# Pearbiossom-M/FlashAttention-from-Scratch-with-Triton

Measured on AMD Instinct MI355X. Metric: achieved TFLOPS fwd and fwd+bwd (B=4,H=32,N=4096,D=64 causal); %MFMA peak, higher is better.
Workload: dtype bf16

## Files before the change

### flashattention-from-scratch-with-triton_amd/csrc/fa_fwd_v4.hip

```cpp
#include <stdlib.h>

#include <type_traits>

#include "fa_common.h"
#include "fa_kernels.h"

namespace fa {

template <int D_>
struct Fwd4Cfg {
  static constexpr int D = D_;
  static constexpr int BM = 256, NT = 256, NW = 4;
  static constexpr int BN = D == 64 ? 128 : 64;
  static constexpr int NBUF = D == 64 ? 3 : 4;
  static constexpr int NKB = BN / 32;
  static constexpr int ROWB = D * 2, CPR = D / 8, KS = D / 16, DB = D / 32;
  static constexpr int TILE_BYTES = BN * ROWB;
  static constexpr int V_BASE = NBUF * TILE_BYTES;
  static constexpr int FLAG_OFF = 2 * NBUF * TILE_BYTES;
  static constexpr int RB_BYTES = 32 * ROWB;
  static constexpr int QS_OFF = FLAG_OFF + 16;
  static constexpr int QS_BYTES = D == 64 ? 8 * RB_BYTES : 0;
  static constexpr int LDS_BYTES = QS_OFF + QS_BYTES;
  static constexpr int PIECES = TILE_BYTES / (NW * 1024);
  static constexpr int RPI = 1024 / ROWB;
  static constexpr int PVG = 2 * DB;
  static constexpr int NSS = 2 * KS, NPV = 2 * PVG, NSLOT = NSS + NPV;
  static constexpr int INFLIGHT = (NBUF - 3) * 2 * PIECES;
};

template <typename T> struct Fwd4Limit;
template <> struct Fwd4Limit<BF16> { static constexpr float value = 1.2676506e30f; };
template <> struct Fwd4Limit<FP16> { static constexpr float value = 32768.0f; };

#ifdef FA_STAMPS
#define FA4_STAMP(slot)                                                           \
  do {                                                                            \
    __builtin_amdgcn_sched_barrier(0);                                            \
    unsigned long long now_;                                                      \
    asm volatile("s_memtime %0\n\ts_waitcnt lgkmcnt(0)" : "=s"(now_)::"memory"); \
    __builtin_amdgcn_sched_barrier(0);                                            \
    seg[slot] += now_ - last_;                                                    \
    last_ = now_;                                                                 \
  } while (0)
#else
#define FA4_STAMP(slot) do {} while (0)
#endif

template <int D, typename T, bool CAUSAL>
__global__ __launch_bounds__(256, 1) void fa_fwd4_kernel(FwdParams p) {
#ifdef FA_STAMPS
  unsigned long long clk0_, rt0_;
  asm volatile("s_memtime %0\n\ts_memrealtime %1\n\ts_waitcnt lgkmcnt(0)" : "=s"(clk0_), "=s"(rt0_)::"memory");
  unsigned long long seg[12] = {0, 0, 0, 0, 0, 0, 0, 0, 0, 0, 0, 0};
  unsigned long long last_ = clk0_, ntile_ = 0, npass_ = 0;
#endif
  using C = Fwd4Cfg<D>;
  using vec8 = typename T::vec8;
  constexpr bool FOLD = T::kFoldScale;
  constexpr bool CHAIN_M = FOLD;
  extern __shared__ __attribute__((aligned(16))) char smem_raw[];
  FA_LDS char* smem = (FA_LDS char*)smem_raw;

  const int tid = threadIdx.x;
  const int lane = tid & 63;
  const int wave = __builtin_amdgcn_readfirstlane(tid >> 6);
  const int r = lane & 31, h = lane >> 5;

  const bool CONT = CAUSAL || (p.Sk % C::BN == 0 && p.Sk / C::BN >= C::NBUF - 1);
  constexpr bool STAGEQ = D == 64;
  const bool paired = CAUSAL && p.pair;
  const int nq = p.nq_tiles;
  const int per_bh = paired ? (nq + 1) / 2 : nq;
  const int n_items = per_bh * p.B * p.H;
  const int Sq = p.Sq, Sk = p.Sk;
  struct Work {
    int b, h, idx, npass;
  };
  auto decode = [&](int item) __attribute__((always_inline)) -> Work {
    const int w = xcd_remap(item, n_items);
    const int bh = p.div_per_bh.div(w), idx = w - bh * per_bh, b = p.div_h.div(bh);
    return Work{b, bh - b * p.H, idx, (paired && idx != nq - 1 - idx) ? 2 : 1};
  };
  auto tile_of = [&](const Work& wk, int pass) __attribute__((always_inline)) -> int {
    return paired ? (pass == 0 ? nq - 1 - wk.idx : wk.idx) : (CAUSAL ? nq - 1 - wk.idx : wk.idx);
  };

  const int q_rs = p.lq.rs, kv_rs = p.lk.rs, o_rs = p.lo.rs;
  auto rsrc_q = [&](const Work& wk, bool valid) __attribute__((always_inline)) {
    return make_rsrc((const char*)p.q + wk.b * p.lq.sb + wk.h * p.lq.sh, valid ? view_bytes(Sq, q_rs, C::ROWB) : 0u);
  };
  auto rsrc_k = [&](const Work& wk, bool valid) __attribute__((always_inline)) {
    return make_rsrc((const char*)p.k + wk.b * p.lk.sb + wk.h * p.lk.sh, valid ? view_bytes(Sk, kv_rs, C::ROWB) : 0u);
  };
  auto rsrc_v = [&](const Work& wk, bool valid) __attribute__((always_inline)) {
    return make_rsrc((const char*)p.v + wk.b * p.lv.sb + wk.h * p.lv.sh, valid ? view_bytes(Sk, kv_rs, C::ROWB) : 0u);
  };

  int dma_src[C::PIECES];
#pragma unroll
  for (int i = 0; i < C::PIECES; ++i) {
    const int row = (C::BN / C::NW) * wave + C::RPI * i + lane / C::CPR;
    dma_src[i] = row * kv_rs + swz_chunk<D>(row, lane % C::CPR) * 16 - 1024 * (i & 1);
  }
  int k_off[C::KS];
#pragma unroll
  for (int ks = 0; ks < C::KS; ++ks) k_off[ks] = lds_off<D>(r, 2 * ks + h);
  int v_off[2][C::DB];
#pragma unroll
  for (int e = 0; e < 2; ++e)
#pragma unroll
    for (int db = 0; db < C::DB; ++db) v_off[e][db] = tr_lane_off<D>(lane, 8 * e, db);
  const float c2 = p.scale * kLog2e;

  if (Sk % C::BN != 0) {
    lds_zero_fill(smem, C::FLAG_OFF, C::NT, tid);
    __syncthreads();
  }

  if (tid == 0) *(FA_LDS int*)(smem + C::FLAG_OFF) = 0;
  bool primed = false;
  int r0 = 0;

  int item = blockIdx.x, pass = 0;
  Work wk = decode(item);
  Work nwk_item = decode(min(item + (int)gridDim.x, n_items - 1));
  for (;;) {
    const int b_ = wk.b, h_ = wk.h;
    const __amdgpu_buffer_rsrc_t rk = rsrc_k(wk, true), rv = rsrc_v(wk, true);
    const __amdgpu_buffer_rsrc_t ro = make_rsrc((char*)p.o + b_ * p.lo.sb + h_ * p.lo.sh, view_bytes(Sq, o_rs, C::ROWB));
    const __amdgpu_buffer_rsrc_t rl = make_rsrc(p.lse + b_ * p.lse_sb + h_ * p.lse_sh, (unsigned)Sq * 4);
    const bool more_pass = pass + 1 < wk.npass, more_item = item + (int)gridDim.x < n_items;
    const bool has_next = CONT && (more_pass || more_item);
    const Work nwk = more_pass ? wk : nwk_item;
    const int nq0_wg = tile_of(nwk, more_pass ? pass + 1 : 0) * C::BM;

    FA4_STAMP(8);
    const int q0_wg = tile_of(wk, pass) * C::BM;
    const int qw = q0_wg + 32 * wave;
    auto qrow = [&](int rb) __attribute__((always_inline)) { return qw + 128 * rb; };

    const int kv_end = CAUSAL ? min(Sk, q0_wg + C::BM) : Sk;
    const int ntiles = (kv_end + C::BN - 1) / C::BN;
    const int nplain = CAUSAL ? min(Sk / C::BN, q0_wg / C::BN) : Sk / C::BN;

    auto dma_pair_of = [&](const __amdgpu_buffer_rsrc_t& rkx, const __amdgpu_buffer_rsrc_t& rvx, int t, int slot, int j) __attribute__((always_inline)) {
      constexpr int HALF = C::PIECES / 2;
      const int i = 2 * (j % HALF);
      const int dst = slot * C::TILE_BYTES + ((C::BN / C::NW) * wave + C::RPI * i) * C::ROWB;
      if (j < HALF) dma_pieces<2>(rkx, lds_addr_of(smem + dst), dma_src + i, t * C::BN * kv_rs);
      else dma_pieces<2>(rvx, lds_addr_of(smem + C::V_BASE + dst), dma_src + i, t * C::BN * kv_rs);
    };
    auto dma_pair = [&](int t, int slot, int j) __attribute__((always_inline)) { dma_pair_of(rk, rv, t, slot, j); };
    auto fetch_tile = [&](int t, int slot) __attribute__((always_inline)) {
#pragma unroll
      for (int j = 0; j < C::PIECES; ++j) dma_pair(t, slot, j);
    };
    auto stage_q_pair = [&](const __amdgpu_buffer_rsrc_t& rqx, int q0, int rb, int hf) __attribute__((always_inline)) {
      if constexpr (STAGEQ) {
        const int prow = lane >> 3;
        int voff[2];
#pragma unroll
        for (int i = 0; i < 2; ++i) {
          const int row = 8 * (2 * hf + i) + prow;
          voff[i] = (q0 + 128 * rb + 32 * wave + row) * q_rs + swz_chunk<D>(row, lane & 7) * 16 - 1024 * i;
        }
        dma_pieces<2>(rqx, lds_addr_of(smem + C::QS_OFF + (2 * wave + rb) * C::RB_BYTES + 2048 * hf), voff, 0);
      }
    };
    const bool was_primed = primed;
    if (!primed) {
      r0 = 0;
      if constexpr (STAGEQ) {
        const __amdgpu_buffer_rsrc_t rq = rsrc_q(wk, true);
#pragma unroll
        for (int g = 0; g < 4; ++g) stage_q_pair(rq, q0_wg, g >> 1, g & 1);
      }
#pragma unroll
      for (int t = 0; t < C::NBUF - 1; ++t) fetch_tile(t, t);
    }
    FA4_STAMP(9);
    u32x4 qf[2][C::KS];
    if constexpr (STAGEQ) {
      if (!was_primed) __builtin_amdgcn_s_waitcnt(0x0F70 | (((C::NBUF - 1) * 2 * C::PIECES) & 15) | ((((C::NBUF - 1) * 2 * C::PIECES) >> 4) << 14));
      asm volatile("" ::: "memory");
#pragma unroll
      for (int rb = 0; rb < 2; ++rb)
#pragma unroll
        for (int ks = 0; ks < C::KS; ++ks) {
          vec8 q = as_vec8<T>(lds_read16(smem + C::QS_OFF + (2 * wave + rb) * C::RB_BYTES + k_off[ks]));
          if constexpr (FOLD) q = scale_frag<T>(q, c2);
          qf[rb][ks] = __builtin_bit_cast(u32x4, q);
        }
    } else {
      const __amdgpu_buffer_rsrc_t rq = rsrc_q(wk, true);
#pragma unroll
      for (int rb = 0; rb < 2; ++rb)
#pragma unroll
        for (int ks = 0; ks < C::KS; ++ks) {
          vec8 q = as_vec8<T>(buf_load16(rq, (qrow(rb) + r) * q_rs + (2 * ks + h) * 16));
          if constexpr (FOLD) q = scale_frag<T>(q, c2);
          qf[rb][ks] = __builtin_bit_cast(u32x4, q);
        }
    }
    FA4_STAMP(10);
    int mask_base[2];
#pragma unroll
    for (int rb = 0; rb < 2; ++rb) mask_base[rb] = (CAUSAL ? min(qrow(rb) + r, Sk - 1) : Sk - 1) - 4 * h;

    auto commit = [&]() __attribute__((always_inline)) {
      asm volatile("" ::: "memory");
      __builtin_amdgcn_s_waitcnt(0x0F70 | (C::INFLIGHT & 15) | ((C::INFLIGHT >> 4) << 14));
      __builtin_amdgcn_s_barrier();
      asm volatile("" ::: "memory");
    };

    f32x16 S_[2][2];
    f32x16 negm[CHAIN_M ? 2 : 1];
    float mrow[2], nmc[2];
    float l[2];
    u32x4 pk[2][2][2];
    constexpr int KR = C::KS < 4 ? C::KS : 4;
    u32x4 KF[KR];
    vec8 VF[2 * C::DB];
    f32x16 oacc[2][C::DB];
    int thr[2][2];

    auto block_valu = [&](int tau, f32x16 (&X)[2], u32x4 (&PK)[2][2], const int (&TH)[2], auto mask_tag, auto has0_tag) __attribute__((always_inline)) {
      constexpr bool MASK = decltype(mask_tag)::value, HAS0 = decltype(has0_tag)::value;
      auto first_q = [](int t) { return t <= 0 ? 0 : (32 * t + C::NSLOT - 1) / C::NSLOT; };
      auto work = [&](int t, bool exps) __attribute__((always_inline)) {
        if (t < 0 || t >= C::NSLOT) return;
#pragma unroll
        for (int u = 0; u < 2; ++u) {
          const int q = first_q(t) + u;
          if (q >= first_q(t + 1) || q >= 32) continue;
          const int rb = (q >> 3) & 1, e = (q & 7) + 8 * (q >> 4);
          if (rb == 0 && !HAS0) continue;
          if (exps) {
            float x = CHAIN_M ? X[rb][e] : (FOLD ? X[rb][e] + nmc[rb] : __builtin_fmaf(X[rb][e], c2, nmc[rb]));
            if constexpr (MASK) x = (e & 3) + 8 * (e >> 2) > TH[rb] ? -INFINITY : x;
            X[rb][e] = __builtin_amdgcn_exp2f(x);
          } else {
            l[rb] += X[rb][e];
            if (q & 1) {
              const int j = e >> 1;
              PK[rb][j >> 2][j & 3] = pack2<T>(X[rb][e - 1], X[rb][e]);
            }
          }
        }
      };
      work(tau - C::NSS, true);
      work(tau - 1 - C::NSS, false);
    };
    auto block_iter = [&](auto j_tag, auto set_tag, auto mode_tag, auto pst_tag, int kb0, const int (&kc)[C::KS], int kc_imm,
                          const int (&kn)[C::KS], int kn_delta, int kn_imm,
                          const int (&vc)[2][C::DB], int vc_imm, int vp0, int vp1, int vp_imm,
                          auto&& hook) __attribute__((always_inline)) {
      constexpr int J = decltype(j_tag)::value, SET = decltype(set_tag)::value, PSET = SET ^ 1;
      constexpr int MODE = decltype(mode_tag)::value, PST = decltype(pst_tag)::value;
      constexpr bool OWN0 = MODE != 3, PREV0 = PST != 2;
      using OwnMask = std::integral_constant<bool, MODE != 0>;
      using PrevMask = std::integral_constant<bool, PST != 0>;
      if constexpr (MODE != 0) {
        thr[SET][0] = mask_base[0] - kb0;
        thr[SET][1] = MODE == 2 ? (1 << 20) : mask_base[1] - kb0;
      }
#pragma unroll
      for (int s = 0; s < C::NSLOT; ++s) {
        hook(J, s);
        if (s < C::NSS) {
          const int ks = s >> 1, rb = s & 1;
          if (rb == 1 || OWN0) {
            if (ks == 0) {
              if constexpr (CHAIN_M) T::mfma_v_first(S_[SET][rb], KF[0], qf[rb][0], negm[CHAIN_M ? rb : 0]);
              else T::mfma_v_first0(S_[SET][rb], KF[0], qf[rb][0]);
            } else {
              T::mfma_v_acc(S_[SET][rb], KF[ks % KR], qf[rb][ks]);
            }
          }
        } else {
          const int n = s - C::NSS, e = n / C::PVG, m = n % C::PVG, rb = m & 1;
          if (rb == 1 || PREV0) oacc[rb][m >> 1] = T::mfma(VF[e * C::DB + (m >> 1)], as_vec8<T>(pk[PSET][rb][e]), oacc[rb][m >> 1]);
        }
        if (s >= 2 && s <= C::NSS && (s & 1) == 0) {
          const int ks = (s - 2) >> 1, nk = ks + KR;
          if (nk < C::KS) KF[ks % KR] = lds_read16(lds_at(kc[nk] + kc_imm));
          else KF[ks % KR] = lds_read16(lds_at(kn[nk - C::KS] + kn_delta + kn_imm));
        }
#pragma unroll
        for (int pp = 0; pp < 2 * C::DB; ++pp) {
          const int e = pp / C::DB, db = pp % C::DB, at = C::NSS + e * C::PVG + 2 * db + 2;
          if (at < C::NSLOT && s == at)
            VF[pp] = lds_read_tr_frag<T>(lds_at(vc[0][db] + vc_imm + 16 * e * C::ROWB), lds_at(vc[1][db] + vc_imm + 16 * e * C::ROWB));
          if (at >= C::NSLOT && s == 0)
            VF[pp] = lds_read_tr_frag<T>(lds_at(vp0 + vp_imm), lds_at(vp1 + vp_imm));
        }
        block_valu(C::NSLOT + s, S_[PSET], pk[PSET], thr[PSET], PrevMask{}, std::integral_constant<bool, PREV0>{});
        block_valu(s, S_[SET], pk[SET], thr[SET], OwnMask{}, std::integral_constant<bool, OWN0>{});
        if constexpr (CHAIN_M) {
          if (s == 1 && OWN0) keep_live(negm[0]);
          if (s == 2) keep_live(negm[CHAIN_M ? 1 : 0]);
        }
        __builtin_amdgcn_sched_barrier(0);
      }
    };
    auto drain = [&](auto set_tag, auto pst_tag, int rt_last) __attribute__((always_inline)) {
      constexpr int PSET = decltype(set_tag)::value ^ 1, PST = decltype(pst_tag)::value;
      constexpr bool PREV0 = PST != 2;
      const int base = C::V_BASE + rt_last * C::TILE_BYTES + (C::NKB - 1) * 32 * C::ROWB + 16 * C::ROWB;
      VF[2 * C::DB - 1] = lds_read_tr_frag<T>(smem + v_off[0][C::DB - 1] + base, smem + v_off[1][C::DB - 1] + base);
#pragma unroll
      for (int s = 0; s < C::NSLOT; ++s) {
        if (s >= C::NSS) {
          const int n = s - C::NSS, e = n / C::PVG, m = n % C::PVG, rb = m & 1;
          if (rb == 1 || PREV0) oacc[rb][m >> 1] = T::mfma(VF[e * C::DB + (m >> 1)], as_vec8<T>(pk[PSET][rb][e]), oacc[rb][m >> 1]);
        }
        block_valu(C::NSLOT + s, S_[PSET], pk[PSET], thr[PSET], std::integral_constant<bool, PST != 0>{}, std::integral_constant<bool, PREV0>{});
        __builtin_amdgcn_sched_barrier(0);
      }
    };

    auto tile_step = [&](int t, int rt, auto mode_tag, auto pst_tag, auto nx_tag) __attribute__((always_inline)) {
      constexpr int MODE = decltype(mode_tag)::value, NX = decltype(nx_tag)::value;
      const __amdgpu_buffer_rsrc_t nrk = rsrc_k(nwk, has_next && NX != 0), nrv = rsrc_v(nwk, has_next && NX != 0);
      const __amdgpu_buffer_rsrc_t nrq = rsrc_q(nwk, has_next && NX == 2);
      using OwnSt = std::integral_constant<int, MODE == 0 ? 0 : (MODE == 3 ? 2 : 1)>;
      const int rn = rt + 1 == C::NBUF ? 0 : rt + 1, rp = rt == 0 ? C::NBUF - 1 : rt - 1;
      const int lds0 = (int)lds_addr_of(smem);
      int kA[C::KS], vA[2][C::DB], vP[2];
      const int kdelta = (rn - rt) * C::TILE_BYTES;
#pragma unroll
      for (int ks = 0; ks < C::KS; ++ks) {
        kA[ks] = opaque(lds0 + k_off[ks] + rt * C::TILE_BYTES);
      }
#pragma unroll
      for (int e = 0; e < 2; ++e) {
#pragma unroll
        for (int db = 0; db < C::DB; ++db) vA[e][db] = opaque(lds0 + v_off[e][db] + C::V_BASE + rt * C::TILE_BYTES);
        vP[e] = opaque(lds0 + v_off[e][C::DB - 1] + C::V_BASE + (t == 0 ? rt * C::TILE_BYTES
                                                                  : rp * C::TILE_BYTES + (C::NKB - 1) * 32 * C::ROWB) + 16 * C::ROWB);
      }
      auto hook = [&](int J, int s) __attribute__((always_inline)) {
        if (J == C::NKB - 1) {
          if (s == 1) commit();
#pragma unroll
          for (int j = 0; j < C::PIECES; ++j)
            if (s == C::NSS + 1 + 2 * j) {
              if constexpr (NX != 0) dma_pair_of(nrk, nrv, t + C::NBUF - 1 - ntiles, rp, j);
              else dma_pair(t + C::NBUF - 1, rp, j);
            }
        }
        if constexpr (NX == 2 && STAGEQ) {
          if (J < 2 && s == C::NSS + 1) stage_q_pair(nrq, nq0_wg, J, 0);
          if (J < 2 && s == C::NSS + 5) stage_q_pair(nrq, nq0_wg, J, 1);
        }
      };
      auto go = [&](auto j_tag) __attribute__((always_inline)) {
        constexpr int J = decltype(j_tag)::value;
        constexpr int kPrevImm = (J - 1) * 32 * C::ROWB + 16 * C::ROWB;
        if constexpr (J == 0)
          block_iter(j_tag, std::integral_constant<int, 0>{}, mode_tag, pst_tag, t * C::BN, kA, 0, kA, 0, 32 * C::ROWB, vA, 0, vP[0], vP[1], 0, hook);
        else if constexpr (J + 1 < C::NKB)
          block_iter(j_tag, std::integral_constant<int, J & 1>{}, mode_tag, OwnSt{}, t * C::BN + 32 * J, kA, J * 32 * C::ROWB, kA, 0,
                     (J + 1) * 32 * C::ROWB, vA, J * 32 * C::ROWB, vA[0][C::DB - 1], vA[1][C::DB - 1], kPrevImm, hook);
        else
          block_iter(j_tag, std::integral_constant<int, J & 1>{}, mode_tag, OwnSt{}, t * C::BN + 32 * J, kA, J * 32 * C::ROWB, kA, kdelta, 0,
                     vA, J * 32 * C::ROWB, vA[0][C::DB - 1], vA[1][C::DB - 1], kPrevImm, hook);
      };
      go(std::integral_constant<int, 0>{});
      go(std::integral_constant<int, 1>{});
      if constexpr (C::NKB == 4) {
        go(std::integral_constant<int, 2>{});
        go(std::integral_constant<int, 3>{});
      }
    };

    auto scout_block = [&](const FA_LDS char* kblk, int kb0, float (&mx)[2]) __attribute__((always_inline)) {
#pragma unroll
      for (int rb = 0; rb < 2; ++rb) {
        f32x16 s;
        T::mfma_v_first0(s, lds_read16(kblk + k_off[0]), qf[rb][0]);
#pragma unroll
        for (int ks = 1; ks < C::KS; ++ks) T::mfma_v_acc(s, lds_read16(kblk + k_off[ks]), qf[rb][ks]);
        settle_mfma(s);
        const int th = opaque(mask_base[rb] - kb0);
        float mm = mx[rb];
#pragma unroll
        for (int i = 0; i < 16; ++i) mm = __builtin_fmaxf(mm, (i & 3) + 8 * (i >> 2) > th ? -INFINITY : s[i]);
        mx[rb] = mm;
      }
    };
    auto set_m = [&](const float (&mx)[2]) __attribute__((always_inline)) {
#pragma unroll
      for (int rb = 0; rb < 2; ++rb) {
        const float m = half_max(mx[rb]);
        mrow[rb] = m > -INFINITY ? m : 0.f;
        nmc[rb] = FOLD ? -mrow[rb] : -mrow[rb] * c2;
        if constexpr (CHAIN_M) {
#pragma unroll
          for (int i = 0; i < 16; ++i) negm[rb][i] = -mrow[rb];
        }
      }
    };

    for (int attempt = 0; attempt < 2; ++attempt) {
      if (attempt == 1) {
        r0 = 0;
#pragma unroll
        for (int t = 0; t < C::NBUF - 1; ++t) fetch_tile(t, t);
      }
      if (!was_primed || attempt == 1) {
        asm volatile("" ::: "memory");
        __builtin_amdgcn_s_waitcnt(0x0070 | (((C::NBUF - 2) * 2 * C::PIECES) & 15) | ((((C::NBUF - 2) * 2 * C::PIECES) >> 4) << 14));
        __builtin_amdgcn_s_barrier();
        asm volatile("" ::: "memory");
      }

      FA4_STAMP(0);
      float mx[2] = {-INFINITY, -INFINITY};
      if (attempt == 0) {
        scout_block(smem + r0 * C::TILE_BYTES, 0, mx);
        set_m(mx);
      } else {
        for (int t = 0; t < ntiles; ++t) {
          if (t > 0) {
            __syncthreads();
            fetch_tile(t, t % C::NBUF);
            __builtin_amdgcn_s_waitcnt(0x0070);
            __syncthreads();
          }
          for (int j = 0; j < C::NKB; ++j)
            scout_block(smem + (t % C::NBUF) * C::TILE_BYTES + j * 32 * C::ROWB, t * C::BN + 32 * j, mx);
        }
        set_m(mx);
        __builtin_amdgcn_s_waitcnt(0x0070);
        __syncthreads();
#pragma unroll
        for (int t = 0; t < C::NBUF - 1; ++t) fetch_tile(t, t);
        asm volatile("" ::: "memory");
        __builtin_amdgcn_s_waitcnt(0x0070 | (((C::NBUF - 2) * 2 * C::PIECES) & 15) | ((((C::NBUF - 2) * 2 * C::PIECES) >> 4) << 14));
        __builtin_amdgcn_s_barrier();
        asm volatile("" ::: "memory");
      }

      FA4_STAMP(1);
#pragma unroll
      for (int rb = 0; rb < 2; ++rb) {
        l[rb] = 0.f;
#pragma unroll
        for (int i = 0; i < 16; ++i) {
          const int q = (i >> 3) * 16 + rb * 8 + (i & 7);
          S_[1][rb][i] = C::NSS + q * C::NSLOT / 32 < C::NSLOT ? 0.f : -INFINITY;
        }
#pragma unroll
        for (int e = 0; e < 2; ++e) pk[1][rb][e] = u32x4{0u, 0u, 0u, 0u};
#pragma unroll
        for (int db = 0; db < C::DB; ++db)
#pragma unroll
          for (int i = 0; i < 16; ++i) oacc[rb][db][i] = 0.f;
        thr[0][rb] = thr[1][rb] = 1 << 20;
      }
#pragma unroll
      for (int ks = 0; ks < KR; ++ks) KF[ks] = lds_read16(smem + r0 * C::TILE_BYTES + k_off[ks]);
#pragma unroll
      for (int pp = 0; pp < 2 * C::DB; ++pp) VF[pp] = as_vec8<T>(u32x4{0u, 0u, 0u, 0u});
      __builtin_amdgcn_sched_barrier(0);

      FA4_STAMP(2);
      int t = 0, rt = r0;
      using I0 = std::integral_constant<int, 0>;
      using I1 = std::integral_constant<int, 1>;
      using I2 = std::integral_constant<int, 2>;
      using I3 = std::integral_constant<int, 3>;
      const int nloop = (!CAUSAL && CONT) ? nplain - (C::NBUF - 1) : nplain;
      for (; t < nloop; ++t, rt = rt + 1 == C::NBUF ? 0 : rt + 1) tile_step(t, rt, I0{}, I0{}, I0{});
#ifdef FA_STAMPS
      FA4_STAMP(3);
      ntile_ += nplain;
      ++npass_;
#endif
      constexpr int RT = 256 / C::BN;
      auto nxt = [](int x) __attribute__((always_inline)) { return x + 1 == C::NBUF ? 0 : x + 1; };
      if constexpr (CAUSAL) {
        int rt_last;
        if constexpr (RT == 2) {
          tile_step(t, rt, I2{}, I1{}, I2{});
          tile_step(t + 1, rt_last = nxt(rt), I3{}, I1{}, I1{});
        } else {
          tile_step(t, rt, I2{}, I1{}, I0{});
          tile_step(t + 1, nxt(rt), I2{}, I1{}, I1{});
          tile_step(t + 2, nxt(nxt(rt)), I3{}, I1{}, I1{});
          tile_step(t + 3, rt_last = nxt(nxt(nxt(rt))), I3{}, I2{}, I1{});
        }
        static_assert(C::NBUF - 1 == (RT == 2 ? 2 : 3), "the masked tiles carry exactly the next pass's first NBUF - 1 tiles");
        FA4_STAMP(4);
        drain(I0{}, I2{}, rt_last);
        rt = rt_last;
      } else {
        if (CONT) {
          if constexpr (C::NBUF == 3) {
            tile_step(t, rt, I0{}, I0{}, I2{});
            tile_step(t + 1, nxt(rt), I0{}, I0{}, I1{});
            rt = nxt(nxt(rt));
          } else {
            tile_step(t, rt, I0{}, I0{}, I1{});
            tile_step(t + 1, nxt(rt), I0{}, I0{}, I1{});
            tile_step(t + 2, nxt(nxt(rt)), I0{}, I0{}, I1{});
            rt = nxt(nxt(nxt(rt)));
          }
          t += C::NBUF - 1;
        }
        for (; t < ntiles; ++t, rt = nxt(rt)) tile_step(t, rt, I1{}, I1{}, I0{});
        rt = rt == 0 ? C::NBUF - 1 : rt - 1;
        FA4_STAMP(4);
        drain(I0{}, I1{}, rt);
      }
      FA4_STAMP(5);

      float lt[2];
      bool bad = false;
#pragma unroll
      for (int rb = 0; rb < 2; ++rb) {
        lt[rb] = half_sum(l[rb]);
        bad = bad || !(lt[rb] <= Fwd4Limit<T>::value);
      }
      FA_LDS int* flag = (FA_LDS int*)(smem + C::FLAG_OFF);
      if (attempt == 0 && __builtin_amdgcn_ballot_w64(bad) != 0 && lane == 0) *flag = 1;
      if (CONT) __builtin_amdgcn_s_waitcnt(0x0070 | (((C::NBUF - 2) * 2 * C::PIECES) & 15) | ((((C::NBUF - 2) * 2 * C::PIECES) >> 4) << 14));
      else __builtin_amdgcn_s_waitcnt(0x0070);
      __syncthreads();
      const int redo = __builtin_amdgcn_readfirstlane(*flag);
      FA4_STAMP(6);
      if (!redo) {
        FA_LDS char* stage = smem + (wave >> 1) * C::V_BASE + rt * C::TILE_BYTES + (wave & 1) * 32 * C::ROWB;
#pragma unroll
        for (int rb = 0; rb < 2; ++rb) {
          const float inv = lt[rb] > 0.f ? 1.0f / lt[rb] : 0.f;
          store_tile_rows<D, T>(oacc[rb], inv, stage, ro, qrow(rb) * o_rs, lane, o_rs);
          if (h == 0)
            buf_store_f32(rl, (qrow(rb) + r) * 4, mrow[rb] * (FOLD ? kLn2 : p.scale) + __builtin_logf(lt[rb]));
        }
        FA4_STAMP(7);
        primed = has_next;
        r0 = rt + 1 == C::NBUF ? 0 : rt + 1;
        break;
      }
      __builtin_amdgcn_s_waitcnt(0x0F70);
      __syncthreads();
      if (tid == 0) {
        *flag = 0;
#ifndef FA_STAMPS
        if (p.dbg) atomicAdd((unsigned*)p.dbg, 1u);
#endif
      }
    }
    if (more_pass) {
      ++pass;
    } else {
      item += gridDim.x;
      if (item >= n_items) break;
      wk = nwk_item;
      nwk_item = decode(min(item + (int)gridDim.x, n_items - 1));
      pass = 0;
    }
  }
#ifdef FA_STAMPS
  if (p.dbg && lane == 0) {
    unsigned long long* d = (unsigned long long*)p.dbg + ((size_t)blockIdx.x * 4 + wave) * 16;
    for (int i = 0; i < 12; ++i) d[i] = seg[i];
    d[12] = npass_;
    d[13] = ntile_;
    unsigned long long clk1_, rt1_;
    asm volatile("s_memtime %0\n\ts_memrealtime %1\n\ts_waitcnt lgkmcnt(0)" : "=s"(clk1_), "=s"(rt1_)::"memory");
    d[14] = clk1_ - clk0_;
    d[15] = rt1_ - rt0_;
  }
#endif
}

template <int D, typename T, bool CAUSAL>
static hipError_t launch4(const FwdParams& p, hipStream_t s) {
  using C = Fwd4Cfg<D>;
  int grid = (CAUSAL && p.pair ? (p.nq_tiles + 1) / 2 : p.nq_tiles) * p.B * p.H;
  if (CAUSAL || (p.Sk % C::BN == 0 && p.Sk / C::BN >= C::NBUF - 1)) {
    static std::atomic<int> cus{0};
    int n = cus.load(std::memory_order_relaxed);
    if (n == 0) {
      int dev = 0;
      if (hipGetDevice(&dev) != hipSuccess || hipDeviceGetAttribute(&n, hipDeviceAttributeMultiprocessorCount, dev) != hipSuccess || n < 8) n = 256;
      n -= n % 8;
      cus.store(n, std::memory_order_relaxed);
    }
    if (grid > n) grid = n;
  }
  auto kern = fa_fwd4_kernel<D, T, CAUSAL>;
  static std::atomic<unsigned long long> opted_in{0};
  if (hipError_t e = opt_in_lds((const void*)kern, C::LDS_BYTES, opted_in)) return e;
  hipLaunchKernelGGL(kern, dim3(grid), dim3(C::NT), C::LDS_BYTES, s, p);
  return hipGetLastError();
}

hipError_t launch_fwd_v4(FwdParams p, int D, int dtype, int causal, hipStream_t s) {
  p.nq_tiles = (p.Sq + 255) / 256;
  p.pair = causal != 0;
  p.div_per_bh = make_fastdiv(p.pair ? (p.nq_tiles + 1) / 2 : p.nq_tiles);
  p.div_h = make_fastdiv(p.H);
#define FA_GO(DD, TT) (causal ? launch4<DD, TT, true>(p, s) : launch4<DD, TT, false>(p, s))
  if (D == 64) return dtype == 1 ? FA_GO(64, BF16) : FA_GO(64, FP16);
  if (D == 128) return dtype == 1 ? FA_GO(128, BF16) : FA_GO(128, FP16);
#undef FA_GO
  return hipErrorInvalidValue;
}

}
```

Measured before the change: 898.2.

## Rebalance causal diagonal work across waves with mirrored row blocks for D=64

For causal D=64, each wave now owns row blocks `wave` and `7-wave` instead of `wave` and `wave+4`, so every wave carries an equal share of diagonal-tile work. A dedicated diagonal phase walks the 32-key sub-blocks per wave, masking only at the diagonal and skipping the work above it. The phase also issues the next pass's K/V tile and Q staging prefetch in its early slots, and the rest after the epilogue. This adds a large amount of per-wave specialised code and changes the prefetch and wait accounting, which risks more register pressure and scheduling fragility.

```diff
diff --git a/flashattention-from-scratch-with-triton_amd/csrc/fa_fwd_v4.hip b/flashattention-from-scratch-with-triton_amd/csrc/fa_fwd_v4.hip
--- a/flashattention-from-scratch-with-triton_amd/csrc/fa_fwd_v4.hip
+++ b/flashattention-from-scratch-with-triton_amd/csrc/fa_fwd_v4.hip
@@ -69,6 +69,7 @@
 
   const bool CONT = CAUSAL || (p.Sk % C::BN == 0 && p.Sk / C::BN >= C::NBUF - 1);
   constexpr bool STAGEQ = D == 64;
+  constexpr bool DIAG = CAUSAL && D == 64;
   const bool paired = CAUSAL && p.pair;
   const int nq = p.nq_tiles;
   const int per_bh = paired ? (nq + 1) / 2 : nq;
@@ -138,7 +139,10 @@
     FA4_STAMP(8);
     const int q0_wg = tile_of(wk, pass) * C::BM;
     const int qw = q0_wg + 32 * wave;
-    auto qrow = [&](int rb) __attribute__((always_inline)) { return qw + 128 * rb; };
+    auto qrow = [&](int rb) __attribute__((always_inline)) {
+      if constexpr (DIAG) return q0_wg + 32 * (rb == 0 ? wave : 7 - wave);
+      else return qw + 128 * rb;
+    };
 
     const int kv_end = CAUSAL ? min(Sk, q0_wg + C::BM) : Sk;
     const int ntiles = (kv_end + C::BN - 1) / C::BN;
@@ -163,7 +167,8 @@
 #pragma unroll
         for (int i = 0; i < 2; ++i) {
           const int row = 8 * (2 * hf + i) + prow;
-          voff[i] = (q0 + 128 * rb + 32 * wave + row) * q_rs + swz_chunk<D>(row, lane & 7) * 16 - 1024 * i;
+          const int rb0 = DIAG ? 32 * (rb == 0 ? wave : 7 - wave) : 128 * rb + 32 * wave;
+          voff[i] = (q0 + rb0 + row) * q_rs + swz_chunk<D>(row, lane & 7) * 16 - 1024 * i;
         }
         dma_pieces<2>(rqx, lds_addr_of(smem + C::QS_OFF + (2 * wave + rb) * C::RB_BYTES + 2048 * hf), voff, 0);
       }
@@ -305,18 +310,62 @@
         __builtin_amdgcn_sched_barrier(0);
       }
     };
-    auto drain = [&](auto set_tag, auto pst_tag, int rt_last) __attribute__((always_inline)) {
+    auto drain = [&](auto set_tag, auto pst_tag, int rt_last, auto vf_tag) __attribute__((always_inline)) {
       constexpr int PSET = decltype(set_tag)::value ^ 1, PST = decltype(pst_tag)::value;
-      constexpr bool PREV0 = PST != 2;
-      const int base = C::V_BASE + rt_last * C::TILE_BYTES + (C::NKB - 1) * 32 * C::ROWB + 16 * C::ROWB;
-      VF[2 * C::DB - 1] = lds_read_tr_frag<T>(smem + v_off[0][C::DB - 1] + base, smem + v_off[1][C::DB - 1] + base);
+      constexpr bool PREV0 = PST < 2, PMASK = PST == 1 || PST == 2 || (PST == 3 && !CHAIN_M);
+      if constexpr (decltype(vf_tag)::value) {
+        const int base = C::V_BASE + rt_last * C::TILE_BYTES + (C::NKB - 1) * 32 * C::ROWB + 16 * C::ROWB;
+        VF[2 * C::DB - 1] = lds_read_tr_frag<T>(smem + v_off[0][C::DB - 1] + base, smem + v_off[1][C::DB - 1] + base);
+      }
 #pragma unroll
       for (int s = 0; s < C::NSLOT; ++s) {
         if (s >= C::NSS) {
           const int n = s - C::NSS, e = n / C::PVG, m = n % C::PVG, rb = m & 1;
           if (rb == 1 || PREV0) oacc[rb][m >> 1] = T::mfma(VF[e * C::DB + (m >> 1)], as_vec8<T>(pk[PSET][rb][e]), oacc[rb][m >> 1]);
         }
-        block_valu(C::NSLOT + s, S_[PSET], pk[PSET], thr[PSET], std::integral_constant<bool, PST != 0>{}, std::integral_constant<bool, PREV0>{});
+        block_valu(C::NSLOT + s, S_[PSET], pk[PSET], thr[PSET], std::integral_constant<bool, PMASK>{}, std::integral_constant<bool, PREV0>{});
+        __builtin_amdgcn_sched_barrier(0);
+      }
+    };
+    auto phase_iter = [&](auto set_tag, auto kind_tag, auto pk_tag, const int (&kn)[C::KS], int kn_delta, int kn_imm,
+                          const int (&vc)[2][C::DB], int vc_imm, auto&& hook) __attribute__((always_inline)) {
+      constexpr int SET = decltype(set_tag)::value, PSET = SET ^ 1, KIND = decltype(kind_tag)::value, PK = decltype(pk_tag)::value;
+      constexpr bool OWN0 = KIND < 2, PREV0 = PK < 2;
+      using OwnMask = std::integral_constant<bool, !CHAIN_M && (KIND == 1 || KIND == 3)>;
+      using PrevMask = std::integral_constant<bool, !CHAIN_M && (PK == 1 || PK == 3)>;
+#pragma unroll
+      for (int s = 0; s < C::NSLOT; ++s) {
+        hook(s);
+        if (s < C::NSS) {
+          const int ks = s >> 1, rb = s & 1;
+          if (rb == 1 || OWN0) {
+            if (ks == 0) {
+              if constexpr (CHAIN_M) T::mfma_v_first(S_[SET][rb], KF[0], qf[rb][0], negm[CHAIN_M ? rb : 0]);
+              else T::mfma_v_first0(S_[SET][rb], KF[0], qf[rb][0]);
+            } else {
+              T::mfma_v_acc(S_[SET][rb], KF[ks % KR], qf[rb][ks]);
+            }
+          }
+        } else {
+          const int n = s - C::NSS, e = n / C::PVG, m = n % C::PVG, rb = m & 1;
+          if (rb == 1 || PREV0) oacc[rb][m >> 1] = T::mfma(VF[e * C::DB + (m >> 1)], as_vec8<T>(pk[PSET][rb][e]), oacc[rb][m >> 1]);
+        }
+        if (KIND != 3 && s >= 2 && s <= C::NSS && (s & 1) == 0) {
+          const int ks = (s - 2) >> 1;
+          KF[ks % KR] = lds_read16(lds_at(kn[ks] + kn_delta + kn_imm));
+        }
+#pragma unroll
+        for (int pp = 0; pp < 2 * C::DB; ++pp) {
+          const int e = pp / C::DB, db = pp % C::DB, at = C::NSS + e * C::PVG + 2 * db + 2;
+          if (s == (at < C::NSLOT ? at : C::NSLOT - 1))
+            VF[pp] = lds_read_tr_frag<T>(lds_at(vc[0][db] + vc_imm + 16 * e * C::ROWB), lds_at(vc[1][db] + vc_imm + 16 * e * C::ROWB));
+        }
+        block_valu(C::NSLOT + s, S_[PSET], pk[PSET], thr[PSET], PrevMask{}, std::integral_constant<bool, PREV0>{});
+        block_valu(s, S_[SET], pk[SET], thr[SET], OwnMask{}, std::integral_constant<bool, OWN0>{});
+        if constexpr (CHAIN_M) {
+          if (s == 1 && OWN0) keep_live(negm[0]);
+          if (s == 2) keep_live(negm[CHAIN_M ? 1 : 0]);
+        }
         __builtin_amdgcn_sched_barrier(0);
       }
     };
@@ -482,20 +531,100 @@
 #endif
       constexpr int RT = 256 / C::BN;
       auto nxt = [](int x) __attribute__((always_inline)) { return x + 1 == C::NBUF ? 0 : x + 1; };
-      if constexpr (CAUSAL) {
+      if constexpr (DIAG) {
+        static_assert(C::NBUF == 3 && RT == 2 && C::KS == KR, "the phase: two 128-key tiles resident, one slot to spare");
+        const int b0 = rt, b1 = nxt(b0), b2 = nxt(b1);
+        {
+          const int base = C::V_BASE + (t == 0 ? b0 * C::TILE_BYTES : b2 * C::TILE_BYTES + (C::NKB - 1) * 32 * C::ROWB) + 16 * C::ROWB;
+          VF[2 * C::DB - 1] = lds_read_tr_frag<T>(smem + v_off[0][C::DB - 1] + base, smem + v_off[1][C::DB - 1] + base);
+        }
+        asm volatile("" ::: "memory");
+        __builtin_amdgcn_s_waitcnt(0x0070);
+        __builtin_amdgcn_s_barrier();
+        asm volatile("" ::: "memory");
+        const __amdgpu_buffer_rsrc_t nrk = rsrc_k(nwk, has_next), nrv = rsrc_v(nwk, has_next), nrq = rsrc_q(nwk, has_next);
+        auto hook_w = [&](int s) __attribute__((always_inline)) {
+#pragma unroll
+          for (int j = 0; j < C::PIECES; ++j)
+            if (s == 1 + 2 * j) dma_pair_of(nrk, nrv, 0, b2, j);
+#pragma unroll
+          for (int g = 0; g < 4; ++g)
+            if (s == C::NSS + 1 + 2 * g) stage_q_pair(nrq, nq0_wg, g >> 1, g & 1);
+        };
+        auto no_hook = [](int) __attribute__((always_inline)) {};
+        auto diag_start = [&](auto set_tag, int rb, int kb0) __attribute__((always_inline)) {
+          const int th = opaque(mask_base[rb] - kb0);
+          if constexpr (CHAIN_M) {
+#pragma unroll
+            for (int i = 0; i < 16; ++i) negm[CHAIN_M ? rb : 0][i] = (i & 3) + 8 * (i >> 2) > th ? -INFINITY : negm[CHAIN_M ? rb : 0][i];
+            settle_mfma(negm[CHAIN_M ? rb : 0]);
+          } else {
+            thr[decltype(set_tag)::value][rb] = th;
+            thr[decltype(set_tag)::value][rb ^ 1] = 1 << 20;
+          }
+        };
+        const int lds0 = (int)lds_addr_of(smem);
+        int kA[C::KS], vA[2][C::DB];
+        auto set_bases = [&](int slot) __attribute__((always_inline)) {
+#pragma unroll
+          for (int ks = 0; ks < C::KS; ++ks) kA[ks] = opaque(lds0 + k_off[ks] + slot * C::TILE_BYTES);
+#pragma unroll
+          for (int e = 0; e < 2; ++e)
+#pragma unroll
+            for (int db = 0; db < C::DB; ++db) vA[e][db] = opaque(lds0 + v_off[e][db] + C::V_BASE + slot * C::TILE_BYTES);
+        };
+        const int kdelta = (b1 - b0) * C::TILE_BYTES;
+        set_bases(b0);
+        auto phase = [&](auto w_tag) __attribute__((always_inline)) {
+          constexpr int W = decltype(w_tag)::value;
+          auto kind_of = [](int c) { return c < W ? 0 : c == W ? 1 : c < 7 - W ? 2 : 3; };
+          auto visit = [&](auto c_tag) __attribute__((always_inline)) {
+            constexpr int Cc = decltype(c_tag)::value, J = Cc % C::NKB;
+            if constexpr (Cc <= 7 - W) {
+              constexpr int KIND = kind_of(Cc), PK = Cc == 0 ? 0 : kind_of(Cc - 1);
+              using Set = std::integral_constant<int, Cc & 1>;
+              if constexpr (Cc == C::NKB) set_bases(b1);
+              if constexpr (KIND == 1) {
+                FA4_STAMP(4);
+                diag_start(Set{}, 0, q0_wg + 32 * Cc);
+                phase_iter(Set{}, std::integral_constant<int, KIND>{}, std::integral_constant<int, PK>{}, kA, J == C::NKB - 1 ? kdelta : 0,
+                           J == C::NKB - 1 ? 0 : (J + 1) * 32 * C::ROWB, vA, J * 32 * C::ROWB, hook_w);
+                FA4_STAMP(11);
+              } else {
+                if constexpr (KIND == 3) diag_start(Set{}, 1, q0_wg + 32 * Cc);
+                phase_iter(Set{}, std::integral_constant<int, KIND>{}, std::integral_constant<int, PK>{}, kA, J == C::NKB - 1 ? kdelta : 0,
+                           J == C::NKB - 1 ? 0 : (J + 1) * 32 * C::ROWB, vA, J * 32 * C::ROWB, no_hook);
+              }
+            }
+          };
+          visit(std::integral_constant<int, 0>{});
+          visit(std::integral_constant<int, 1>{});
+          visit(std::integral_constant<int, 2>{});
+          visit(std::integral_constant<int, 3>{});
+          visit(std::integral_constant<int, 4>{});
+          visit(std::integral_constant<int, 5>{});
+          visit(std::integral_constant<int, 6>{});
+          visit(std::integral_constant<int, 7>{});
+          FA4_STAMP(4);
+          drain(std::integral_constant<int, ((7 - W) & 1) ^ 1>{}, I3{}, 0, std::false_type{});
+        };
+        switch (wave) {
+          case 0: phase(I0{}); break;
+          case 1: phase(I1{}); break;
+          case 2: phase(I2{}); break;
+          default: phase(I3{}); break;
+        }
+        rt = b1;
+      } else if constexpr (CAUSAL) {
+        static_assert(RT == 4, "D = 128: four 64-key tiles level with the query tile");
         int rt_last;
-        if constexpr (RT == 2) {
-          tile_step(t, rt, I2{}, I1{}, I2{});
-          tile_step(t + 1, rt_last = nxt(rt), I3{}, I1{}, I1{});
-        } else {
-          tile_step(t, rt, I2{}, I1{}, I0{});
-          tile_step(t + 1, nxt(rt), I2{}, I1{}, I1{});
-          tile_step(t + 2, nxt(nxt(rt)), I3{}, I1{}, I1{});
-          tile_step(t + 3, rt_last = nxt(nxt(nxt(rt))), I3{}, I2{}, I1{});
-        }
-        static_assert(C::NBUF - 1 == (RT == 2 ? 2 : 3), "the masked tiles carry exactly the next pass's first NBUF - 1 tiles");
+        tile_step(t, rt, I2{}, I1{}, I0{});
+        tile_step(t + 1, nxt(rt), I2{}, I1{}, I1{});
+        tile_step(t + 2, nxt(nxt(rt)), I3{}, I1{}, I1{});
+        tile_step(t + 3, rt_last = nxt(nxt(nxt(rt))), I3{}, I2{}, I1{});
+        static_assert(C::NBUF - 1 == 3, "the masked tiles carry exactly the next pass's first NBUF - 1 tiles");
         FA4_STAMP(4);
-        drain(I0{}, I2{}, rt_last);
+        drain(I0{}, I2{}, rt_last, std::true_type{});
         rt = rt_last;
       } else {
         if (CONT) {
@@ -514,7 +643,7 @@
         for (; t < ntiles; ++t, rt = nxt(rt)) tile_step(t, rt, I1{}, I1{}, I0{});
         rt = rt == 0 ? C::NBUF - 1 : rt - 1;
         FA4_STAMP(4);
-        drain(I0{}, I1{}, rt);
+        drain(I0{}, I1{}, rt, std::true_type{});
       }
       FA4_STAMP(5);
 
@@ -527,12 +656,20 @@
       }
       FA_LDS int* flag = (FA_LDS int*)(smem + C::FLAG_OFF);
       if (attempt == 0 && __builtin_amdgcn_ballot_w64(bad) != 0 && lane == 0) *flag = 1;
-      if (CONT) __builtin_amdgcn_s_waitcnt(0x0070 | (((C::NBUF - 2) * 2 * C::PIECES) & 15) | ((((C::NBUF - 2) * 2 * C::PIECES) >> 4) << 14));
+      if constexpr (DIAG) __builtin_amdgcn_s_waitcnt(0x0070);
+      else if (CONT) __builtin_amdgcn_s_waitcnt(0x0070 | (((C::NBUF - 2) * 2 * C::PIECES) & 15) | ((((C::NBUF - 2) * 2 * C::PIECES) >> 4) << 14));
       else __builtin_amdgcn_s_waitcnt(0x0070);
       __syncthreads();
       const int redo = __builtin_amdgcn_readfirstlane(*flag);
       FA4_STAMP(6);
       if (!redo) {
+        if constexpr (DIAG) {
+          static_assert(C::INFLIGHT == 0, "the next pass's first commit counts nothing: the epilogue's stores may lie behind tile 1");
+          const __amdgpu_buffer_rsrc_t nrk = rsrc_k(nwk, has_next), nrv = rsrc_v(nwk, has_next);
+          const int b0 = rt == 0 ? C::NBUF - 1 : rt - 1;
+#pragma unroll
+          for (int j = 0; j < C::PIECES; ++j) dma_pair_of(nrk, nrv, 1, b0, j);
+        }
         FA_LDS char* stage = smem + (wave >> 1) * C::V_BASE + rt * C::TILE_BYTES + (wave & 1) * 32 * C::ROWB;
 #pragma unroll
         for (int rb = 0; rb < 2; ++rb) {
```

New measurement: 899.5, median of 5. About the same (+0.1%).
